# david-mathews-1994/deltarice

Measured on AMD Instinct MI355X. Metric: encode+decode GB/s (int16 in), higher is better.
Workload: dtype int16; 1 GPU; 1000000x7000 int16 Gaussian(sigma=10), m=8, 500 chunks of 2000x7000 per GPU, encode then decode, HBM resident; waveforms_per_gpu=1000000, wave_len=7000, rice_m=8, chunks_per_gpu=500, decode_impl=8

## Files before the change

### deltarice_amd/csrc/drx_blocks.hip

```cpp
#include <hip/hip_runtime.h>
#include <stdint.h>
#include <type_traits>

#include "drx_device.h"
#include "drx_internal.h"
#include "drx_iir_math.h"

namespace drx {

constexpr int kBlkSegWMin = 9;
__host__ __device__ constexpr int blk_segw_plan(uint32_t k) { return k <= 4u ? 11 : (k <= 7u ? 15 : 19); }
__host__ __device__ constexpr int blk_segw_bits10(uint64_t b10) { return b10 >= 117u ? 19 : (b10 >= 82u ? 15 : (b10 >= 54u ? 11 : 9)); }
__host__ __device__ constexpr uint32_t blk_lane_cap(int segw) { return segw <= 11 ? 76u : (segw == 15 ? 68u : 60u); }
constexpr uint32_t kBlkPre = 8;
constexpr uint32_t kBlkGuessBits = 128;
constexpr uint32_t kBlkRounds = 8;
constexpr uint32_t kBlkTail = 4;

template <int NT, int SW>
struct BlkGeom {
    static constexpr int kSegW = SW;
    static constexpr uint32_t kLaneCap = blk_lane_cap(SW);
    static constexpr uint32_t kLaneStride = kLaneCap / 2u + 1u;
    static constexpr uint32_t kWords = NT * SW;
// ... 607 lines not shown
                }
            };
            const bool lane_ok = cnt <= kBlkLaneCap && todo == cnt;
            if (!wg_any(!lane_ok)) {
                constexpr int NR = (int)(kBlkLaneCap / 2u);
                uint32_t rr[NR];
                const uint32_t wmax = (uint32_t)__builtin_amdgcn_readfirstlane((int)wave_max_u32(cnt));
#pragma unroll
                for (int i = 0; i < NR; ++i) {
                    rr[i] = 0;
                    if (2u * (uint32_t)i < wmax) rr[i] = my_stage[i];
                }
                if (RESID) s_e[tid] = sum;
                blk_barrier();
                const uint32_t base16 = RESID ? 0u : (acc_base + pre_s + incl_s - sum) & 0xffffu;
                typedef uint16_t u16x2 __attribute__((ext_vector_type(2)));
                const u16x2 b2 = {(uint16_t)base16, (uint16_t)base16};
                uint16_t *const op = obuf + (a0 + rel0);
                {
                    const uint32_t o = a0 + rel0;
                    const bool odd = (o & 1u) != 0u;
                    uint32_t *const dp = reinterpret_cast<uint32_t *>(obuf) + (o >> 1);
                    const uint32_t sel = odd ? 0x05040302u : 0x07060504u;
                    const uint32_t lim = cnt == 0u ? 0u : (odd ? cnt : cnt - 1u);
                    uint32_t prevp = RESID ? (tid ? s_e[tid - 1u] << 16 : 0u) : __builtin_bit_cast(uint32_t, b2);
#pragma unroll
                    for (int i = 0; i < NR; ++i) {
                        if (2u * (uint32_t)i < wmax) {
                            const uint32_t cur = __builtin_bit_cast(uint32_t, (u16x2)(__builtin_bit_cast(u16x2, rr[i]) + b2));
                            const uint32_t d = __builtin_amdgcn_perm(cur, prevp, sel);
                            if (2u * (uint32_t)i < lim) dp[i] = d;
                            prevp = cur;
                        }
                    }
                    if (cnt != 0u) op[cnt - 1u] = (uint16_t)(base16 + sum);
                }
                blk_barrier();
                if (FUSE) iir_lds(a0, blk_count);
                copy_out(0u);
            } else {
                uint32_t c = 0, acc = acc_base + pre_s + incl_s - sum;
                Qp = C - (todo ? f : B0);
                for (uint32_t R0 = 0; R0 < blk_count; R0 += BG::kOutCap) {
                    const uint32_t cmax = (rel0 >= R0 + BG::kOutCap) ? 0u : ((todo < R0 + BG::kOutCap - rel0) ? todo : R0 + BG::kOutCap - rel0);
                    uint16_t *outp = obuf + (int32_t)(a0 + rel0 - R0);
                    blk_parse<kBlkValue, RESID>(W, k, c < cmax, Qp, 0u, c, acc, cmax, outp);
                    blk_barrier();
                    if (FUSE) iir_lds(a0, (blk_count - R0 < BG::kOutCap) ? blk_count - R0 : BG::kOutCap);
                    copy_out(R0);
                    blk_barrier();
                }
            }
            if (FUSE && last_of_run && tid == 0u)
                __hip_atomic_store(xstate + sidx, (1ull << 63) | (uint64_t)(xs.x & 0xffffu) | ((uint64_t)(xs.y & 0xffffu) << 16) | ((uint64_t)(xs.z & 0xffffu) << 32),
                                   __ATOMIC_RELAXED, __HIP_MEMORY_SCOPE_AGENT);
            blk_barrier();
        }
        if (next_unit >= total_units) return;
        unit = next_unit;
        cur = nxt;
    }
}

static int nt_for_len(uint32_t wave_len, uint32_t k) {
    const uint64_t typ_words = ((uint64_t)wave_len * (2u * k + 7u)) >> 6;
    return typ_words <= blk_words(64, k) ? 64 : (typ_words <= blk_words(128, k) ? 128 : 256);
}
static int blocks_nt(const Geom &G) { return G.uniform ? nt_for_len(G.u_wave_len, G.k) : (int)G.rag_blk_nt; }

static double blocks_weighted(uint64_t waves, uint32_t wave_len, uint32_t k, int nt) {
    const uint64_t typ_words = ((uint64_t)wave_len * (2u * k + 7u)) >> 6;
    const uint64_t bpw = (typ_words + blk_words((uint32_t)nt, k) - 1u) / blk_words((uint32_t)nt, k);
    return (double)(waves * bpw) * (bpw <= 2u ? 1.7 : 1.0);
}
static double blocks_us_of(double weighted_blocks, int nt, uint32_t k) {
    const double resident = nt == 256 ? 768.0 : (nt == 128 ? 1536.0 : 3072.0);
    const double t_blk = (nt == 256 ? 21.0 : (nt == 128 ? 28.0 : 41.0)) * (double)blk_segw_plan(k) / 11.0;
    return (double)(uint64_t)((weighted_blocks + resident - 1.0) / resident) * t_blk;
}

bool blocks_batch(const Geom &G) {
    if (G.n_taps != 0 && !G.fast_taps) return false;
    if (!G.uniform) return G.rag_blocks != 0;
    if (!(G.total_waves <= 98304u && G.u_wave_len >= 2048u)) return false;
    const int nt = blocks_nt(G);
    const uint64_t typ_words = ((uint64_t)G.u_wave_len * (2u * G.k + 7u)) >> 6;
    const uint64_t bpw = (typ_words + blk_words((uint32_t)nt, G.k) - 1u) / blk_words((uint32_t)nt, G.k);
    const double blocks_us = blocks_us_of((double)(G.total_waves * bpw), nt, G.k) * (bpw <= 2u ? 1.7 : 1.0);
    const double lanes_us = 0.06 * (double)G.u_wave_len * (double)((G.total_waves + 98303u) / 98304u);
    return blocks_us < lanes_us;
}

std::vector<uint32_t> blocks_plan_ragged(Geom &G, const ChunkDesc *d) {
    G.rag_blocks = 0;
    G.rag_blk_classes = 0;
    uint32_t max_len = 0, min_len = 0xffffffffu;
    for (uint64_t c = 0; c < G.n_chunks; ++c) {
        max_len = d[c].wave_len > max_len ? d[c].wave_len : max_len;
        min_len = d[c].wave_len < min_len ? d[c].wave_len : min_len;
    }
    if (G.total_waves > 98304u || min_len < 2048u) return {};
    const int nt = nt_for_len(max_len, G.k);
    double wb = 0;
    for (uint64_t c = 0; c < G.n_chunks; ++c) wb += blocks_weighted(d[c].n_waves, d[c].wave_len, G.k, nt);
    const double lanes_us = 0.06 * (double)max_len * (double)((G.total_waves + 98303u) / 98304u);
    if (!(blocks_us_of(wb, nt, G.k) < lanes_us)) return {};
    const uint64_t per = (max_payload_words(max_len) + blk_words_min(64u) - 1u) / blk_words_min(64u);
    if (G.total_waves * per * 12u > (1ull << 30)) return {};
    G.rag_blocks = 1u;
    G.rag_blk_nt = (uint32_t)nt;
    G.rag_blk_slots = (uint32_t)(per ? per : 1u);
    std::vector<uint32_t> list(G.total_waves);
    uint32_t n_cls = 0, at = 0;
    for (int b = 31; b >= 11; --b) {
        uint32_t cnt = 0, cls_max = 0;
        for (uint64_t c = 0; c < G.n_chunks; ++c) {
            if ((31 - __builtin_clz(d[c].wave_len)) != b) continue;
            for (uint32_t i = 0; i < d[c].n_waves; ++i) list[at + cnt++] = (uint32_t)(d[c].wave_base + i);
            cls_max = d[c].wave_len > cls_max ? d[c].wave_len : cls_max;
        }
        if (!cnt) continue;
        G.rag_blk_class_off[n_cls] = at;
        G.rag_blk_class_len[n_cls] = cls_max;
        at += cnt;
        ++n_cls;
    }
    G.rag_blk_class_off[n_cls] = at;
    G.rag_blk_classes = n_cls;
    return list;
}

uint32_t blocks_iir_tab_words() { return 3u * kRunTabWords; }
void blocks_iir_tables(const uint32_t fast_nt[3], uint32_t t0neg, uint32_t *tab) {
    iir_run_tables(fast_nt, t0neg, 76u, tab);
    iir_run_tables(fast_nt, t0neg, 68u, tab + kRunTabWords);
    iir_run_tables(fast_nt, t0neg, 60u, tab + 2u * kRunTabWords);
}

static uint32_t blocks_slots_per_wave(const Geom &G) {
    if (!G.uniform) return G.rag_blk_slots;
    const uint64_t per = (max_payload_words(G.u_wave_len) + blk_words_min(blocks_nt(G)) - 1u) / blk_words_min(blocks_nt(G));
    return (uint32_t)(per ? per : 1u);
}

constexpr uint32_t kBlkMaxClasses = 32;
struct BlkScratch {
    uint32_t *info, *fail, *suspect, *ticket, *ends;
    uint64_t *state, *xstate;
    uint64_t bytes;
};
static BlkScratch blocks_layout(const Geom &G, void *base) {
    const uint64_t W = G.total_waves, U = W * blocks_slots_per_wave(G);
    uint64_t n32 = 4u * kBlkMaxClasses + W + W + 1u;
    n32 = (n32 + 3u) & ~3ull;
    BlkScratch L;
    uint32_t *p = reinterpret_cast<uint32_t *>(base);
    L.info = p;
    L.fail = p + 4u * kBlkMaxClasses;
    L.suspect = L.fail + W;
    L.ticket = L.suspect + W;
    L.ends = p + n32;
    const uint64_t ends32 = (U + 1u) & ~1ull;
    L.state = reinterpret_cast<uint64_t *>(L.ends + ends32);
    L.xstate = L.state + U;
    L.bytes = (n32 + ends32) * 4u + 2u * U * 8u;
    return L;
}

uint64_t blocks_scratch_bytes(const Geom &G) { return blocks_batch(G) ? blocks_layout(G, nullptr).bytes : 0; }

hipError_t launch_decode_blocks(const Geom &G, const uint32_t *d_in, uint64_t in_words, const uint64_t *d_wave_off,
                                const uint32_t *d_wave_words, void *d_blk, DevStatus *d_status, int16_t *d_out,
                                const uint32_t **fail_out, const uint32_t **suspect_out, bool resid, hipStream_t s, bool *fused_out) {
    const BlkScratch L = blocks_layout(G, d_blk);
    hipError_t e = hipMemsetAsync(d_blk, 0, L.bytes, s);
    if (e != hipSuccess) return e;
    const uint32_t spw = blocks_slots_per_wave(G);
    const uint64_t b10 = G.total_samples ? 320ull * in_words / G.total_samples : 65ull;
    const int sw = blk_segw_bits10(b10);
    auto resident_of = [](int nt) { return 256u * (nt == 64 ? 12u : (nt == 128 ? 6u : 3u)); };
    auto nt_gen = [](int nt) { return nt < 128 ? 128 : nt; };
    bool fuse = resid && G.blk_iir_tab != nullptr && !(G.dbg & DRX_DBG_IIR_SEPARATE);
    if (fuse) {
        if (G.uniform) fuse = G.total_waves >= resident_of(nt_gen(blocks_nt(G)));
        else
            for (uint32_t c = 0; c < G.rag_blk_classes; ++c)
                fuse = fuse && (G.rag_blk_class_off[c + 1] - G.rag_blk_class_off[c]) >= resident_of(nt_gen(nt_for_len(G.rag_blk_class_len[c], G.k)));
    }
// ... 53 lines not shown
```

### deltarice_amd/csrc/drx_decode_kernels.hip

```cpp
#include <hip/hip_runtime.h>
#include <stdint.h>

#include <algorithm>
#include <type_traits>

#include "drx_internal.h"
#include "drx_device.h"
#include "drx_walk.h"

namespace drx {

__global__ __launch_bounds__(64) void k_decode_simple(Geom G, const uint32_t *__restrict__ in,
                                                      const uint64_t *__restrict__ wave_off,
                                                      const uint32_t *__restrict__ wave_words, DevStatus *st,
                                                      int16_t *__restrict__ out, const uint32_t *__restrict__ only) {
    const uint64_t g = (uint64_t)blockIdx.x * 64u + threadIdx.x;
    if (g >= G.total_waves) return;
    if (only && !only[g]) return;
    const WaveRef r = locate(G, g);
    const uint32_t *s = in + wave_off[g] + 1;
    const uint32_t n = wave_words[g];
    int16_t *y = out + r.sample_off;
    const uint32_t k = G.k;
    uint64_t win = 0;
// ... 94 lines not shown
                const uint32_t s2 = sacc + d;
                if (EMIT) {
                    if (act && idx + c < len) {
                        const uint32_t i = idx + c;
                        if (((i + par4) & 1u) == 0u) {
                            held = s2 & 0xffffu;
                            held_i = i;
                            holding = true;
                        } else if (holding) {
                            *reinterpret_cast<uint32_t *>(y + i - 1u) = held | (s2 << 16);
                            holding = false;
                        } else {
                            y[i] = (int16_t)(uint16_t)s2;
                        }
                    }
                }
                sacc = act ? s2 : sacc;
                Q = act ? Q + nu : Q;
                c += act ? 1u : 0u;
            }
        }
        if (EMIT && holding) y[held_i] = (int16_t)(uint16_t)held;
        const uint32_t pos = 0u - Q;
        end = pos;
        cnt = c;
        sum = sacc;
    };

    while (done < len && blk_word < n) {
#pragma unroll
        for (int rr = 0; rr < kLongSeg; ++rr) {
            const uint32_t j = tid + NT * (uint32_t)rr;
            const uint32_t wvl = (blk_word + j < n) ? src[blk_word + j] : 0u;
            const uint32_t sgm = j / kLongSeg, i = j % kLongSeg;
            col[(kLongRows - 2u - i) * NT + sgm] = wvl;
            if (i < (uint32_t)kLongOv && sgm >= 1u) col[(kLongRows - 2u - ((uint32_t)kLongSeg + i)) * NT + sgm - 1u] = wvl;
        }
        if (tid < (uint32_t)kLongOv) {
            const uint32_t wi = blk_word + NT * kLongSeg + tid;
            col[(kLongRows - 2u - ((uint32_t)kLongSeg + tid)) * NT + NT - 1u] = (wi < n) ? src[wi] : 0u;
        }
        __syncthreads();
        const uint32_t seg_word = blk_word + tid * kLongSeg;
        const uint32_t avail_bits = seg_word < n ? ((n - seg_word) > (1u << 26) ? 0xffffffffu : (n - seg_word) * 32u) : 0u;

        uint32_t start = tid == 0 ? carry_in : kLongSegBits - kLongGuessBits, end, cnt, sum;
        parse(true, start, avail_bits, std::false_type{}, 0u, 0u, end, cnt, sum);
        for (uint32_t it = 0; it < NT; ++it) {
            s_end[tid] = end;
            __syncthreads();
            const uint32_t pe = tid ? s_end[tid - 1u] : 0u;
            const uint32_t ns = tid == 0 ? carry_in : (pe >= kLongSegBits ? pe - kLongSegBits : kLongSegBits);
            const bool changed = ns != start;
            if (!__syncthreads_or(changed ? 1 : 0)) break;
            start = ns;
            uint32_t e2, c2, s2;
            parse(changed, start, avail_bits, std::false_type{}, 0u, 0u, e2, c2, s2);
            if (changed) { end = e2; cnt = c2; sum = s2; }
        }
        const uint32_t incl_c = wave_incl_scan_dpp(cnt), incl_s = wave_incl_scan_dpp(sum);
        if (lane == 63) { s_tot[0][wv] = incl_c; s_tot[1][wv] = incl_s; }
        s_end[tid] = end;
        __syncthreads();
        uint32_t pre_c = 0, pre_s = 0, tot_c = 0, tot_s = 0;
#pragma unroll
        for (int i = 0; i < kLongWaves; ++i) {
            const uint32_t tc = s_tot[0][i], ts = s_tot[1][i];
            if (i < wv) { pre_c += tc; pre_s += ts; }
            tot_c += tc;
            tot_s += ts;
        }
        const uint32_t end_last = s_end[NT - 1u];
        uint32_t e3, c3, s3;
        parse(true, start, avail_bits, std::true_type{}, done + pre_c + incl_c - cnt, acc_base + pre_s + incl_s - sum, e3, c3, s3);
        done = (tot_c > len - done) ? len : done + tot_c;
        acc_base += tot_s;
        carry_in = end_last >= kLongSegBits ? end_last - kLongSegBits : 0u;
        blk_word += NT * kLongSeg;
        __syncthreads();
    }
    if (done < len && tid == 0) atomicOr(&st->err, kErrCorrupt);
}

template <bool FUSED, bool GEN = false>
__global__ __launch_bounds__(64, 1) void k_decode_lanes(Geom G, const uint32_t *__restrict__ in, uint64_t in_words,
                                                     const uint64_t *__restrict__ chunk_word_off,
                                                     uint64_t *__restrict__ wave_off,
                                                     uint32_t *__restrict__ wave_words,
                                                     uint64_t *__restrict__ granules, uint32_t *__restrict__ ticket,
                                                     DevStatus *st, int16_t *__restrict__ out) {
    constexpr int RW = 64;
    constexpr int LW = 16;
    constexpr int T = 64;
    constexpr int GS = 16;
    constexpr int LOG_RW = 6;
    constexpr int OSW = T / 2 + 4;
    constexpr int PPS = T / 8;
    constexpr int SPI = 64 / PPS;
    constexpr int NV = LW / 4;
    constexpr uint32_t WMASK = (1u << 27) - 1u;
    constexpr uint32_t NEED_AT = GS + 2;
    static_assert(T % GS == 0 && RW - LW >= GS + 2, "round length / ring slack");
    __shared__ uint32_t ring_all[(RW + 2) * 64];
    uint32_t *const ring = ring_all + 64;
    __shared__ __attribute__((aligned(16))) uint32_t obuf[64 * OSW];
    uint64_t *tab_off = reinterpret_cast<uint64_t *>(obuf);
    uint32_t *tab_lo = obuf + 128, *tab_hi = obuf + 192;
    static_assert(64 * OSW >= 256, "tables fit in obuf");

    const int lane = lane_id();
    const uint32_t k = G.k;
    typedef uint32_t u32x4v __attribute__((ext_vector_type(4)));
    typedef u32x4v __attribute__((address_space(1))) g_uint4;
    typedef int16_t __attribute__((address_space(1))) g_i16;
    g_i16 *const outg = (g_i16 *)out;
    uint64_t g;
    bool active;
    uint32_t len = 0, n = 0;
    uint64_t S = 1, ooff = 0;
    [[maybe_unused]] const uint32_t &len_ = len;
    const uint32_t wave_idx = blockIdx.x;
    if (FUSED) {
        uint32_t tk = 0;
        if (lane == 0) tk = atomicAdd(ticket, 1u);
        tk = (uint32_t)__builtin_amdgcn_readfirstlane((int)tk);
        constexpr bool kBlockWalkFits = sizeof(ring_all) >= kWalkBlockWords * 4u && sizeof(obuf) >= kWalkHopCap * 8u;
        const bool u_short = G.uniform && G.u_wave_len <= kWalkShortLen;
        const uint32_t n_blockwalk = G.uniform ? (u_short ? (uint32_t)G.n_chunks : 0u) : G.n_short;
        const uint64_t n_chain = G.uniform ? (u_short ? 0ull : G.n_chunks) : (uint64_t)G.n_long;
        const uint32_t n_walk = n_blockwalk + (uint32_t)((n_chain + (uint32_t)kWalkChains - 1u) / (uint32_t)kWalkChains);
        if (tk < n_walk) {
            __builtin_amdgcn_s_setprio(3);
            if (tk < n_blockwalk) {
                if constexpr (kBlockWalkFits) {
                    const uint64_t c = G.uniform ? (uint64_t)tk : (uint64_t)G.walk_short[tk];
                    walk_chunk_block(G, c, in, in_words, chunk_word_off, wave_off, wave_words, granules, st, ring_all,
                                     reinterpret_cast<uint2 *>(obuf));
                }
            } else {
                walk_chunks_scalar(G, (uint64_t)(tk - n_blockwalk) * kWalkChains, G.uniform ? nullptr : G.walk_long, n_chain,
                                   in, in_words, chunk_word_off, wave_off, wave_words, granules, st);
            }
            return;
        }
        const uint64_t t2 = tk - n_walk;
        uint64_t grp = t2 / G.n_chunks, c = t2 - grp * G.n_chunks;
        uint32_t idx = (uint32_t)grp * 64u + lane;
        uint64_t gr = 0;
        if (G.uniform) {
            const uint32_t full = G.u_n_waves >> 6, rem = G.u_n_waves & 63u;
            const uint64_t t_full = (uint64_t)full * G.n_chunks;
            if (t2 < t_full) {
                active = true;
            } else {
                if (rem == 0u) return;
                const uint32_t per = 64u / rem, sub = (uint32_t)lane / rem;
                const uint64_t c0 = (t2 - t_full) * per;
                if (c0 >= G.n_chunks) return;
                c = c0 + sub;
                idx = full * 64u + ((uint32_t)lane - sub * rem);
                active = sub < per && c < G.n_chunks;
                if (!active) { c = c0; idx = 0; }
            }
            g = c * G.u_n_waves + idx;
            if (active) {
                len = (idx + 1 == G.u_n_waves) ? (G.u_n_samples - idx * G.u_wave_len) : G.u_wave_len;
                ooff = c * (uint64_t)G.u_n_samples + (uint64_t)idx * G.u_wave_len;
            }
        } else {
            const ChunkDesc d = G.chunks[c];
            if ((uint32_t)grp * 64u >= d.n_waves) return;
            active = idx < d.n_waves;
            g = d.wave_base + idx;
            if (active) {
                len = (idx + 1 == d.n_waves) ? (d.n_samples - idx * d.wave_len) : d.wave_len;
                ooff = d.sample_off + (uint64_t)idx * d.wave_len;
            }
        }
        uint32_t spins = 0;
        for (;;) {
            if (active && !(gr & kGranValid))
                gr = __hip_atomic_load(granules + g, __ATOMIC_RELAXED, __HIP_MEMORY_SCOPE_AGENT);
            if (!__any(active && !(gr & kGranValid))) break;
            __builtin_amdgcn_s_sleep(8);
            if (++spins > (1u << 24)) {
                if (lane == 0) atomicOr(&st->err, kErrInternal);
                gr |= kGranValid;
                break;
            }
        }
        if (active) {
            n = (uint32_t)(gr >> 32) & 0x7fffffffu;
            S = chunk_word_off[c] + (uint32_t)gr + 1u;
        }
    } else if (!G.uniform && G.rag_order) {
        if (wave_idx >= G.rag_groups) return;
        const uint2 e = G.rag_order[wave_idx];
        const ChunkDesc d = G.chunks[e.x];
        const uint32_t idx = e.y * 64u + (uint32_t)lane;
        active = idx < d.n_waves;
        g = d.wave_base + idx;
        if (active) {
            len = (idx + 1 == d.n_waves) ? (d.n_samples - idx * d.wave_len) : d.wave_len;
            ooff = d.sample_off + (uint64_t)idx * d.wave_len;
            S = wave_off[g] + 1u;
            n = wave_words[g];
        }
    } else {
        g = (uint64_t)wave_idx * 64u + lane;
        active = g < G.total_waves;
        if (active) {
            const WaveRef r = locate(G, g);
            len = r.len;
            ooff = r.sample_off;
            S = wave_off[g] + 1u;
            n = wave_words[g];
        }
    }
    const uint32_t phi = active ? (uint32_t)((((uintptr_t)out >> 1) + ooff) & (uint64_t)(T - 1)) : 0u;
    const uint32_t steps = wave_max_u32(len + phi);
    const uint32_t lo_max = wave_max_u32(phi);
    const uint32_t hi_min = ~wave_max_u32(~(phi + len));
    uint64_t wo_off[PPS];
    uint32_t wo_lo[PPS], wo_hi[PPS];
    tab_off[lane] = ooff - phi;
    tab_lo[lane] = phi;
    tab_hi[lane] = phi + len;
    wave_sync();
#pragma unroll
    for (int i = 0; i < PPS; ++i) {
        const int st = i * SPI + lane / PPS, p = lane % PPS;
        wo_off[i] = tab_off[st] + 8u * (uint32_t)p;
        wo_lo[i] = tab_lo[st];
        wo_hi[i] = tab_hi[st];
    }
    wave_sync();

    const uint64_t A = (S & ~(uint64_t)(RW - 1)) - (uint64_t)RW;
    const uint32_t s0 = (uint32_t)(S - A);
    const uint32_t endw = s0 + n;
    uint32_t flw = s0 & ~(uint32_t)(LW - 1);
    const bool in_vec_ok = ((uintptr_t)in & 15u) == 0;
    uint32_t *myring = ring + lane;
    typedef uint16_t __attribute__((may_alias)) u16a;
    u16a *myout = reinterpret_cast<u16a *>(obuf + lane * OSW);
    auto store16 = [&](g_i16 *dst, const uint4 &v) __attribute__((always_inline)) {
        *(g_uint4 *)dst = (u32x4v){v.x, v.y, v.z, v.w};
    };
    auto orow16 = [&](int st, int p) __attribute__((always_inline)) -> uint4 {
        return *reinterpret_cast<const uint4 *>(obuf + st * OSW + 4 * p);
    };

    auto load_piece = [&](uint4 (&v)[NV], uint32_t ahead = 0) {
        const uint64_t a = A + flw + ahead;
        if (in_vec_ok && a + (uint32_t)LW <= in_words) {
#pragma unroll
            for (int j = 0; j < NV; ++j) v[j] = *reinterpret_cast<const uint4 *>(in + a + 4 * j);
        } else {
#pragma unroll
            for (int j = 0; j < NV; ++j) {
                v[j].x = (a + 4 * j + 0 < in_words) ? in[a + 4 * j + 0] : 0u;
                v[j].y = (a + 4 * j + 1 < in_words) ? in[a + 4 * j + 1] : 0u;
                v[j].z = (a + 4 * j + 2 < in_words) ? in[a + 4 * j + 2] : 0u;
                v[j].w = (a + 4 * j + 3 < in_words) ? in[a + 4 * j + 3] : 0u;
            }
        }
    };
    auto store_piece = [&](const uint4 (&v)[NV]) {
        const uint32_t r0 = (uint32_t)RW - (flw & (uint32_t)(RW - 1));
        uint32_t *dst = myring + r0 * 64u;
#pragma unroll
        for (int j = 0; j < NV; ++j) {
            dst[-(4 * j + 0) * 64] = v[j].x; dst[-(4 * j + 1) * 64] = v[j].y;
            dst[-(4 * j + 2) * 64] = v[j].z; dst[-(4 * j + 3) * 64] = v[j].w;
        }
        if (r0 == (uint32_t)RW) {
            myring[0] = v[0].x;
            myring[-64] = v[0].y;
        }
        flw += (uint32_t)LW;
    };

    uint32_t Q = 0u - 32u * s0;
    uint32_t Q_need;
    auto set_limits = [&]() __attribute__((always_inline)) {
        const bool more = flw < endw;
        Q_need = more ? ~(32u * (flw - NEED_AT + 1u)) : Q - 0x7fffffffu;
    };
    auto sync_refill = [&]() __attribute__((always_inline)) {
        for (;;) {
            const uint32_t avail = (flw - ((~Q) >> 5)) & WMASK;
            const bool more = flw < endw;
            if (!__any(more && avail < NEED_AT)) break;
            if (more && avail <= (uint32_t)(RW - LW)) {
                uint4 v[NV];
                load_piece(v);
                store_piece(v);
            }
            wave_sync();
        }
    };

    {
        uint4 v[NV];
        for (int i = 0; i < RW / LW; ++i) {
            if (__ballot(flw < endw && flw + (uint32_t)LW <= s0 + (uint32_t)RW) == 0) break;
            if (flw < endw && flw + (uint32_t)LW <= s0 + (uint32_t)RW) {
                load_piece(v);
                store_piece(v);
            }
        }
        wave_sync();
    }
    int32_t acc = 0;
    int32_t y2 = 0, y3 = 0;
    const uint32_t nt1 = GEN ? G.fast_nt[0] & 0xffffu : 0u, nt2 = GEN ? G.fast_nt[1] & 0xffffu : 0u,
                   nt3 = GEN ? G.fast_nt[2] & 0xffffu : 0u;
    const bool t0neg = GEN && G.fast_t0neg;
    auto advance = [&](int32_t d) __attribute__((always_inline)) {
        if constexpr (GEN) {
            uint32_t a = (uint32_t)d + __umul24(nt1, (uint32_t)acc) + __umul24(nt2, (uint32_t)y2) + __umul24(nt3, (uint32_t)y3);
            if (t0neg) a = 0u - a;
            y3 = y2;
            y2 = acc;
            acc = (int32_t)a;
        } else {
            acc += d;
        }
    };

    const uint32_t hi_step = phi + len;
    uint32_t Q_end = 0;
    auto decode_group = [&](auto first_tag, auto edge_tag, int tg, uint32_t tcur) __attribute__((always_inline)) {
        constexpr bool FIRST = decltype(first_tag)::value;
        constexpr bool EDGE = decltype(edge_tag)::value;
        if (!FIRST) {
#pragma unroll
            for (int u = 0; u < GS; u += 2) {
                const uint32_t row = __builtin_amdgcn_ubfe(Q, 5u, (uint32_t)LOG_RW);
                const uint32_t *wp = myring + row * 64u;
                const uint32_t lo = wp[0], hi = wp[64], lo2 = wp[-64];
                const uint32_t winA = __builtin_amdgcn_alignbit(hi, lo, Q);
                const uint32_t winB = __builtin_amdgcn_alignbit(lo, lo2, Q);
                const uint32_t q1 = ffbh(winA);
                const uint32_t kk1 = (winA < (1u << 24)) ? 16u : k;
                const uint32_t nu1 = ~(q1 + kk1);
                const uint32_t win2 = __builtin_amdgcn_alignbit(winA, winB, nu1);
                const uint32_t q2 = ffbh(win2);
                const uint32_t kk2 = (win2 < (1u << 24)) ? 16u : k;
                const uint32_t nu2 = ~(q2 + kk2);
                if constexpr (EDGE) {
                    Q_end = (tcur + (uint32_t)u + 1u == hi_step) ? Q + nu1 : Q_end;
                    Q_end = (tcur + (uint32_t)u + 2u == hi_step) ? Q + nu1 + nu2 : Q_end;
                }
                asm("v_add3_u32 %0, %1, %2, %3" : "=v"(Q) : "v"(Q), "v"(nu1), "v"(nu2));
                const uint32_t z1 = (q1 << kk1) + __builtin_amdgcn_ubfe(winA, nu1, kk1);
                const uint32_t z2 = (q2 << kk2) + __builtin_amdgcn_ubfe(win2, nu2, kk2);
                advance((int32_t)(z1 >> 1) ^ -(int32_t)(z1 & 1u));
                const uint32_t a1 = (uint32_t)acc;
                advance((int32_t)(z2 >> 1) ^ -(int32_t)(z2 & 1u));
                *reinterpret_cast<uint32_t *>(myout + tg + u) = __builtin_amdgcn_perm((uint32_t)acc, a1, 0x05040100u);
            }
            return;
        }
#pragma unroll
        for (int u = 0; u < GS; ++u) {
            const uint32_t row = __builtin_amdgcn_ubfe(Q, 5u, (uint32_t)LOG_RW);
            const uint32_t *wp = myring + row * 64u;
            const uint32_t lo = wp[0], hi = wp[64];
            const uint32_t win = __builtin_amdgcn_alignbit(hi, lo, Q);
            const uint32_t q = ffbh(win);
            const bool esc = win < (1u << 24);
            const uint32_t kk = esc ? 16u : k;
            const uint32_t used = q + kk + 1u;
            const uint32_t rem = __builtin_amdgcn_ubfe(win, 32u - used, kk);
            const uint32_t z = (q << kk) + rem;
            const int32_t d = (int32_t)(z >> 1) ^ -(int32_t)(z & 1u);
            const bool act = (uint32_t)(tg + u) >= phi;
            const int32_t o1 = acc, o2 = y2, o3 = y3;
            advance(d);
            acc = act ? acc : o1;
            y2 = act ? y2 : o2;
            y3 = act ? y3 : o3;
            Q = act ? Q - used : Q;
            if constexpr (EDGE) Q_end = (tcur + (uint32_t)u + 1u == hi_step) ? Q : Q_end;
            myout[tg + u] = (uint16_t)acc;
        }
    };

    auto emit_masked = [&](g_i16 *dst, uint32_t lo, uint32_t hi, uint32_t t0, const uint4 &v) __attribute__((always_inline)) {
        const int p = lane % PPS;
        const uint32_t tpos = t0 + 8u * (uint32_t)p;
        if (tpos + 8u > lo && tpos < hi) {
            if (tpos >= lo && tpos + 8u <= hi) {
                *(g_uint4 *)dst = (u32x4v){v.x, v.y, v.z, v.w};
            } else {
                const uint32_t w[4] = {v.x, v.y, v.z, v.w};
#pragma unroll
                for (int j = 0; j < 8; ++j)
                    if (tpos + (uint32_t)j >= lo && tpos + (uint32_t)j < hi)
                        dst[j] = (int16_t)(w[j >> 1] >> (16 * (j & 1)));
            }
        }
    };
    auto write_out = [&](uint32_t t0) __attribute__((always_inline)) {
        if (t0 >= lo_max && t0 + T <= hi_min) {
#pragma unroll
            for (int i = 0; i < PPS; ++i) {
                const int st = i * SPI + lane / PPS, p = lane % PPS;
                const uint4 v = orow16(st, p);
                store16(outg + wo_off[i] + t0, v);
            }
        } else {
#pragma unroll
            for (int i = 0; i < PPS; ++i) {
                const int st = i * SPI + lane / PPS, p = lane % PPS;
                const uint32_t tpos = t0 + 8u * (uint32_t)p;
                if (tpos + 8u > wo_lo[i] && tpos < wo_hi[i]) emit_masked(outg + wo_off[i] + t0, wo_lo[i], wo_hi[i], t0, orow16(st, p));
            }
        }
    };

    if (steps > 0) {
#pragma unroll 1
        for (int tg = 0; tg < T; tg += GS) {
            sync_refill();
            decode_group(std::true_type{}, std::true_type{}, tg, (uint32_t)tg);
        }
        wave_sync();
        write_out(0);
        wave_sync();
    }

    auto edge_round = [&](uint32_t t0) __attribute__((always_inline)) {
#pragma unroll 1
        for (int tg = 0; tg < T; tg += GS) {
            sync_refill();
            decode_group(std::false_type{}, std::true_type{}, tg, t0 + (uint32_t)tg);
        }
        wave_sync();
        write_out(t0);
        wave_sync();
    };
    uint32_t t0 = T;
    for (; t0 < steps && !(t0 >= lo_max && t0 + T <= hi_min); t0 += T) edge_round(t0);

    const uint32_t min_words = ((uint32_t)T * (k + 1u)) >> 5;
    uint4 pv0[NV], pv1[NV];
    bool pneed0 = false, pneed1 = false;
    set_limits();
    auto group_refill = [&]() __attribute__((always_inline)) {
        if (__any((int32_t)(Q - Q_need) <= 0)) {
            uint32_t avail = (flw - ((~Q) >> 5)) & WMASK;
            if (pneed0 && avail <= (uint32_t)(RW - LW)) {
                store_piece(pv0);
                pneed0 = false;
                avail += (uint32_t)LW;
                if (pneed1 && avail <= (uint32_t)(RW - LW)) { store_piece(pv1); pneed1 = false; }
            }
            if (!pneed0 && pneed1) {
#pragma unroll
                for (int j = 0; j < NV; ++j) pv0[j] = pv1[j];
                pneed0 = true;
                pneed1 = false;
            }
            wave_sync();
            sync_refill();
            set_limits();
        }
    };
    for (; t0 + T <= hi_min && t0 < steps; t0 += T) {
#pragma unroll 1
        for (int tg = 0; tg < T; tg += GS) {
            group_refill();
            decode_group(std::false_type{}, std::false_type{}, tg, 0u);
        }
        Q_end = (t0 + (uint32_t)T == hi_step) ? Q : Q_end;
        wave_sync();
        if (pneed0) store_piece(pv0);
        if (pneed1) store_piece(pv1);
        wave_sync();
        set_limits();
        {
            const uint32_t mc = (t0 + 2u * T <= hi_min && t0 + T < steps) ? min_words : 0u;
            const uint32_t avail = (flw - ((~Q) >> 5)) & WMASK;
            pneed0 = (flw < endw) && avail + (uint32_t)LW <= (uint32_t)RW + mc;
            pneed1 = pneed0 && (flw + (uint32_t)LW < endw) && avail + 2u * (uint32_t)LW <= (uint32_t)RW + mc;
            if (pneed0) load_piece(pv0);
            if (pneed1) load_piece(pv1, (uint32_t)LW);
        }
#pragma unroll
        for (int i = 0; i < PPS; ++i) {
            const int st = i * SPI + lane / PPS, p = lane % PPS;
            const uint4 v = orow16(st, p);
            store16(outg + wo_off[i] + t0, v);
        }
        wave_sync();
    }
    if (pneed0) store_piece(pv0);
    if (pneed1) store_piece(pv1);
    wave_sync();
    for (; t0 < steps; t0 += T) edge_round(t0);
    if (active && len && (((0u - Q_end) - 32u * s0 + 31u) >> 5) != n) atomicOr(&st->err, kErrCorrupt);
}

std::vector<uint2> decode_plan_ragged(Geom &G, const ChunkDesc *d) {
    const uint64_t n = G.n_chunks;
    uint32_t max_groups = 0, max_len = 0;
    for (uint64_t c = 0; c < n; ++c) {
        max_groups = std::max(max_groups, (d[c].n_waves + 63u) / 64u);
        max_len = std::max(max_len, d[c].wave_len);
    }
    G.max_groups = max_groups;
    G.max_wave_len64 = 64ull * max_len;
    std::vector<uint32_t> by_len(n);
    for (uint64_t c = 0; c < n; ++c) by_len[c] = (uint32_t)c;
    std::stable_sort(by_len.begin(), by_len.end(), [&](uint32_t a, uint32_t b) { return d[a].wave_len > d[b].wave_len; });
    std::vector<uint2> order;
    uint64_t n_long_groups = 0;
    for (uint32_t c : by_len)
        for (uint32_t j = 0; j < (d[c].n_waves + 63u) / 64u; ++j) {
            order.push_back(make_uint2(c, j));
            if (d[c].wave_len > kWalkShortLen) ++n_long_groups;
        }
    if (order.size() <= 0x7fffffffull) {
        G.rag_groups = (uint32_t)order.size();
        G.rag_groups_long = (uint32_t)n_long_groups;
    } else {
        order.clear();
    }
    return order;
}

enum class Dec { Simple, Blocks, Long, LanesFused, Lanes, LanesSplit };
enum class Walk { None, InLaunch, Parallel, Serial };
struct DecodeRoute {
    Dec dec;
    Walk walk;
    WalkRoute par;
    bool gen;
};

static DecodeRoute route_decode(const Geom &G, int impl, bool tables_ready, bool have_pw, bool have_blk, bool have_side) {
    DecodeRoute R{};
    R.gen = G.n_taps != 0;
    R.par = route_walk(G, tables_ready, have_pw);
    const bool simple = impl == 0 || (R.gen && !G.fast_taps);
    const bool want_fused = !tables_ready && impl == 8;
    const bool blocks = !simple && !(G.dbg & (DRX_DBG_NO_LONG_PATHS | DRX_DBG_LONG_NOT_BLOCKS)) && have_blk && blocks_batch(G) && (!R.gen || (G.iir_tab && G.iir_state));
    const bool longp = !simple && !blocks && !R.gen && !(G.dbg & DRX_DBG_NO_LONG_PATHS) && G.uniform && long_waveform_batch(G.total_waves, G.u_wave_len);
    const bool sparse = !G.uniform && (uint64_t)G.n_chunks * G.max_groups > 8ull * ((G.total_waves + 63u) / 64u) + 4096ull;
    R.dec = simple ? Dec::Simple : (blocks ? Dec::Blocks : (longp ? Dec::Long : Dec::Lanes));
    const bool parallel = R.par.chunk_wide || R.par.blocks;
    if (R.dec == Dec::Lanes && want_fused && !sparse && !parallel) R.dec = Dec::LanesFused;
    R.walk = tables_ready ? Walk::None : (R.dec == Dec::LanesFused ? Walk::InLaunch : (parallel ? Walk::Parallel : Walk::Serial));
    if (R.dec == Dec::Lanes && R.par.chunk_wide && R.par.blocks && have_side && G.rag_order && G.rag_groups_long &&
        G.rag_groups_long < G.rag_groups && !(G.dbg & DRX_DBG_RAGGED_ONE_LANES_LAUNCH)) R.dec = Dec::LanesSplit;
    return R;
}

hipError_t launch_decode(const Geom &G, const uint32_t *d_in, uint64_t in_words,
                         const uint64_t *d_chunk_word_off, int16_t *d_out, uint64_t *d_wave_off,
                         uint32_t *d_wave_words, uint64_t *d_granules, DevStatus *d_status, int impl, bool tables_ready,
                         void *d_pw, void *d_blk, const SideStream *side, hipEvent_t *ev, hipStream_t s, uint32_t *path_out) {
    uint32_t path_dummy = 0;
    uint32_t &path = path_out ? *path_out : path_dummy;
    path = 0;
    if (G.total_waves == 0) return hipSuccess;
    mark(ev, 0, s);
    const DecodeRoute R = route_decode(G, impl, tables_ready, d_pw != nullptr, d_blk != nullptr, side && side->s);
    const bool gen = R.gen;
    const unsigned nb_plain = blocks_for(G.total_waves, 64);

    auto launch_lanes = [&](const Geom &Gv, unsigned nb, hipStream_t st_) {
        path |= DRX_PATH_LANES;
        if (gen)
            k_decode_lanes<false, true><<<nb, 64, 0, st_>>>(Gv, d_in, in_words, d_chunk_word_off, d_wave_off, d_wave_words, nullptr, nullptr, d_status, d_out);
        else
            k_decode_lanes<false><<<nb, 64, 0, st_>>>(Gv, d_in, in_words, d_chunk_word_off, d_wave_off, d_wave_words, nullptr, nullptr, d_status, d_out);
    };

    if (R.walk == Walk::InLaunch) {
        hipError_t e = hipMemsetAsync(d_granules, 0, (G.total_waves + 2) * sizeof(uint64_t), s);
        if (e != hipSuccess) return e;
    } else if (R.walk == Walk::Parallel) {
        const bool split = R.dec == Dec::LanesSplit;
        hipError_t e = walk_scratch_reset(G, d_pw, s);
        if (e != hipSuccess) return e;
        const bool forked = R.par.chunk_wide && R.par.blocks && side && side->s;
        hipStream_t spw = forked ? side->s : s;
        if (forked) {
            if ((e = hipEventRecord(side->fork, s)) != hipSuccess) return e;
            if ((e = hipStreamWaitEvent(side->s, side->fork, 0)) != hipSuccess) return e;
        }
        if (R.par.chunk_wide)
            launch_walk_chunk_wide(G, d_in, in_words, d_chunk_word_off, d_wave_off, d_wave_words, d_status, d_pw, R.par.by_chains, spw);
        if (split) {
            Geom Gl = G;
            Gl.rag_groups = G.rag_groups_long;
            launch_lanes(Gl, Gl.rag_groups, spw);
        }
        if (forked && (e = hipEventRecord(side->join, side->s)) != hipSuccess) {
            (void)hipStreamSynchronize(side->s);
            return e;
        }
        if (R.par.blocks) launch_walk_blocks(G, d_in, in_words, d_chunk_word_off, d_wave_off, d_wave_words, d_status, d_pw, s);
        if (split) {
            mark(ev, 1, s);
            Geom Gs = G;
            Gs.rag_order = G.rag_order + G.rag_groups_long;
            Gs.rag_groups = G.rag_groups - G.rag_groups_long;
            launch_lanes(Gs, Gs.rag_groups, s);
        }
        if (forked && (e = hipStreamWaitEvent(s, side->join, 0)) != hipSuccess) {
            (void)hipStreamSynchronize(side->s);
            return e;
        }
    } else if (R.walk == Walk::Serial) {
        launch_walk_serial(G, d_in, in_words, d_chunk_word_off, d_wave_off, d_wave_words, d_status, s);
    }
    if (R.dec != Dec::LanesSplit) mark(ev, 1, s);

    switch (R.dec) {
    case Dec::LanesFused: {
        uint32_t *ticket = reinterpret_cast<uint32_t *>(d_granules + G.total_waves);
        unsigned n_walk, groups;
        unsigned nb;
        if (G.uniform) {
            n_walk = (G.u_wave_len <= kWalkShortLen) ? (unsigned)G.n_chunks : blocks_for(G.n_chunks, kWalkChains);
            groups = (G.u_n_waves + 63u) / 64u;
            const uint32_t full = G.u_n_waves >> 6, rem = G.u_n_waves & 63u;
            nb = n_walk + (unsigned)(G.n_chunks * full) + (rem ? (unsigned)((G.n_chunks + 64u / rem - 1u) / (64u / rem)) : 0u);
        } else {
            n_walk = G.n_short + blocks_for(G.n_long, kWalkChains);
            groups = G.max_groups;
            nb = n_walk + (unsigned)(G.n_chunks * groups);
        }
        path |= DRX_PATH_LANES_FUSED;
        if (gen)
            k_decode_lanes<true, true><<<nb, 64, 0, s>>>(G, d_in, in_words, d_chunk_word_off, d_wave_off, d_wave_words, d_granules, ticket, d_status, d_out);
        else
            k_decode_lanes<true><<<nb, 64, 0, s>>>(G, d_in, in_words, d_chunk_word_off, d_wave_off, d_wave_words, d_granules, ticket, d_status, d_out);
        break;
    }
    case Dec::Blocks: {
        const uint32_t *fail = nullptr, *suspect = nullptr;
        bool fused = false;
        hipError_t e = launch_decode_blocks(G, d_in, in_words, d_wave_off, d_wave_words, d_blk, d_status, d_out, &fail, &suspect, gen, s, &fused);
        if (e != hipSuccess) return e;
        path |= DRX_PATH_BLOCKS | (gen ? (fused ? DRX_PATH_IIR_FUSED : DRX_PATH_IIR) : 0u);
        k_decode_long<<<(unsigned)G.total_waves, kLongThreads, 0, s>>>(G, d_in, d_wave_off, d_wave_words, d_status, d_out, fail, suspect, gen ? 1u : 0u);
        if (gen) {
            if (!fused && (e = launch_iir(G, G.iir_chunk_tile_base, G.iir_n_tiles, G.iir_tab, G.iir_state, fail, d_status, d_out, s)) != hipSuccess) return e;
            k_decode_simple<<<nb_plain, 64, 0, s>>>(G, d_in, d_wave_off, d_wave_words, d_status, d_out, fail);
        }
        break;
    }
    case Dec::Long:
        path |= DRX_PATH_LONG;
        k_decode_long<<<(unsigned)G.total_waves, kLongThreads, 0, s>>>(G, d_in, d_wave_off, d_wave_words, d_status, d_out, nullptr, nullptr, 0u);
        break;
    case Dec::Lanes:
// ... 16 lines not shown
```

### deltarice_amd/csrc/drx_internal.h

```cpp
#ifndef DRX_INTERNAL_H
#define DRX_INTERNAL_H

#include <hip/hip_runtime.h>
#include <stdint.h>

#include <vector>

#include "../../include/deltarice_hip.h"

namespace drx {

struct ChunkDesc {
    uint64_t sample_off;
    uint64_t wave_base;
    uint32_t n_samples;
    uint32_t wave_len;
    uint32_t n_waves;
    uint32_t pad_;
};

struct Geom {
    const ChunkDesc *chunks;
    uint64_t n_chunks;
    uint64_t total_waves;
    uint32_t uniform;
    uint32_t u_n_samples, u_wave_len, u_n_waves;
    uint32_t k;
    uint32_t n_taps;
    const int32_t *taps;
    uint32_t fast_taps, fast_t0neg;
    uint32_t fast_nt[3];
    uint32_t enc_fast;
    uint32_t enc_t[4];
    uint64_t total_samples;
    uint64_t *host_words;
    uint32_t dbg;
    const uint32_t *walk_short, *walk_long;
    uint32_t n_short, n_long, max_groups;
    uint64_t max_wave_len64;
    uint32_t rag_blocks, rag_blk_nt, rag_blk_slots;
    const uint32_t *rag_blk_list;
    uint32_t rag_blk_classes;
    uint32_t rag_blk_class_off[33], rag_blk_class_len[32];
    const uint32_t *iir_tab;
    const uint32_t *blk_iir_tab;
    const uint64_t *iir_chunk_tile_base;
    uint64_t iir_n_tiles;
    uint64_t *iir_state;
    const uint64_t *seg_unit_base;
    uint64_t seg_units;
    uint32_t rag_par, rag_bw_blocks_max;
    uint32_t rag_bw_min_len;
    uint32_t rag_pw_min_waves;
    const uint2 *rag_order;
    uint32_t rag_groups;
    uint32_t rag_groups_long;
    const uint32_t *pc_wg_base;
    uint32_t pc_super;
    uint32_t pc_packed;
};

struct DevStatus {
    uint32_t err;
    uint32_t pad_;
    uint64_t total_words;
};

constexpr uint32_t kErrCapacity = 1u;
constexpr uint32_t kErrCorrupt = 2u;
constexpr uint32_t kErrInternal = 4u;

hipError_t launch_encode(const Geom &G, const int16_t *d_in, uint32_t *d_out, uint64_t out_cap,
                         uint64_t *d_chunk_word_off, uint32_t *d_wave_words, uint32_t *d_wave_rel,
                         uint64_t *d_chunk_words, DevStatus *d_status, hipEvent_t *ev, hipStream_t s);

__host__ __device__ inline bool long_waveform_batch(uint64_t total_waves, uint32_t wave_len) {
    return (wave_len >= 65536u && total_waves <= 16384u) || (wave_len >= 16384u && total_waves <= 4096u);
}
static inline unsigned blocks_for(uint64_t items, unsigned per_block) { return (unsigned)((items + per_block - 1) / per_block); }
static inline void mark(hipEvent_t *ev, int i, hipStream_t s) {
    if (ev) (void)hipEventRecord(ev[i], s);
}

inline uint64_t chunk_max_words(uint32_t n_samples, uint32_t n_waves) { return 1u + 2ull * n_waves + (((uint64_t)n_samples * 25u + 31u) >> 5); }

struct WalkRoute {
    bool chunk_wide, blocks;
    bool by_chains;
};
WalkRoute route_walk(const Geom &G, bool tables_ready, bool have_scratch);
std::vector<uint32_t> walk_plan_ragged(Geom &G, const ChunkDesc *host_chunks);
uint64_t walk_scratch_bytes(const Geom &G);
hipError_t walk_scratch_reset(const Geom &G, void *d_pw, hipStream_t s);
void launch_walk_chunk_wide(const Geom &G, const uint32_t *d_in, uint64_t in_words, const uint64_t *d_chunk_word_off,
                            uint64_t *d_wave_off, uint32_t *d_wave_words, DevStatus *d_status, void *d_pw, bool by_chains, hipStream_t s);
void launch_walk_blocks(const Geom &G, const uint32_t *d_in, uint64_t in_words, const uint64_t *d_chunk_word_off,
                        uint64_t *d_wave_off, uint32_t *d_wave_words, DevStatus *d_status, void *d_pw, hipStream_t s);
void launch_walk_serial(const Geom &G, const uint32_t *d_in, uint64_t in_words, const uint64_t *d_chunk_word_off,
                        uint64_t *d_wave_off, uint32_t *d_wave_words, DevStatus *d_status, hipStream_t s);
hipError_t launch_sideband_tables(const Geom &G, const uint32_t *d_in, uint64_t in_words, const uint64_t *d_chunk_word_off,
                                  const uint32_t *d_n, uint64_t *d_wave_off, uint32_t *d_wave_words, DevStatus *d_status, hipStream_t s,
                                  const uint32_t *d_list = nullptr, uint32_t n_list = 0);
int select_walk_class(uint32_t n_waves, uint32_t wave_len);
hipError_t launch_select_walk(const Geom &G, const uint32_t *d_in, uint64_t in_words, const uint64_t *d_chunk_word_off,
                              const uint32_t *d_lists, uint32_t n_sparse, uint32_t n_block, uint32_t n_chain, uint32_t *d_fail,
                              uint64_t *d_wave_off, uint32_t *d_wave_words, DevStatus *d_status, hipStream_t s);
hipError_t launch_decode_select(const Geom &G, const uint32_t *d_in, const uint64_t *d_wave_off, const uint32_t *d_wave_words,
                                const uint64_t *d_sel, uint64_t n_sel, DevStatus *d_status, int16_t *d_out, uint64_t stride,
                                hipStream_t s);
uint64_t gather_scan_blocks(uint64_t n_sel);
hipError_t launch_gather(const Geom &G, const uint32_t *d_in, const uint64_t *d_wave_off, const uint32_t *d_wave_words,
                         const uint64_t *d_sel, uint64_t n_sel, uint64_t chunk_waves, const uint32_t *d_chunk_samples,
                         uint32_t *d_out, uint64_t out_cap, uint64_t *d_out_chunk_off, uint32_t *d_out_wave_words,
                         uint32_t *d_ent_words, uint64_t *d_ent_pos, uint64_t *d_block_sum, uint32_t *d_ctrl, bool tiles,
                         uint64_t mean_words, bool resume, DevStatus *d_status, hipEvent_t *ev, hipStream_t s);
hipError_t launch_estimate_words(const Geom &G, const int16_t *d_in, unsigned long long *d_words16, hipStream_t s);

hipError_t launch_encode_fused(const Geom &G, int wide, const int16_t *d_in, uint32_t *d_out, uint64_t out_cap,
                               uint64_t *d_chunk_word_off, uint32_t *d_wave_words, uint64_t *d_scan,
                               DevStatus *d_status, hipEvent_t *ev, hipStream_t s);

constexpr uint32_t kEsRingWords = 2496;
constexpr uint64_t kEsMinUnits = 8192;
hipError_t launch_encode_stream(const Geom &G, const int16_t *d_in, uint32_t *d_out, uint64_t out_cap,
                                uint64_t *d_chunk_word_off, uint32_t *d_wave_words, uint64_t *d_scan,
                                DevStatus *d_status, hipEvent_t *ev, hipStream_t s);

constexpr uint32_t kEsSegWaves = 4;
constexpr uint32_t kEsSegMinLen = 1024, kEsSegMaxLen = 7168;
struct EsSegShape { uint32_t seg_len, nseg, tpw; };
__host__ __device__ inline EsSegShape es_seg_shape(uint32_t L, uint32_t seg_target) {
    EsSegShape sh;
    uint32_t n = (L + seg_target - 1u) / seg_target;
    n = n ? n : 1u;
    const uint32_t dn = n / kEsSegWaves * kEsSegWaves, up = (n + kEsSegWaves - 1u) / kEsSegWaves * kEsSegWaves;
    n = up;
    if (dn && dn != up) {
        const uint64_t sd = (L + dn - 1u) / dn, su = (L + up - 1u) / up;
        const uint64_t pen_dn = sd > seg_target ? (sd - seg_target) * 55u : 0u, pen_up = su < seg_target ? (seg_target - su) * 40u : 0u;
        if (sd * 57u <= (uint64_t)seg_target * 67u && pen_dn < pen_up) n = dn;
    }
    sh.seg_len = (((L + n - 1u) / n) + 7u) & ~7u;
    sh.nseg = (L + sh.seg_len - 1u) / sh.seg_len;
    sh.tpw = (sh.nseg + kEsSegWaves - 1u) / kEsSegWaves;
    return sh;
}
inline bool stream_segs_admits(const Geom &G) { return G.uniform && (G.n_taps == 0 || G.enc_fast) && G.u_wave_len >= 64u &&
                                                       G.total_waves * es_seg_shape(G.u_wave_len, kEsSegMinLen).tpw < 0xffff0000ull; }
constexpr uint32_t kEsSegsFromLen = 20480;
inline uint64_t segs_scan_words(const Geom &G, uint32_t seg_target) { return 3 * G.total_waves * es_seg_shape(G.u_wave_len, seg_target).tpw + 192; }
hipError_t launch_encode_stream_segs(const Geom &G, uint32_t seg_target, const int16_t *d_in, uint32_t *d_out, uint64_t out_cap,
                                     uint64_t *d_chunk_word_off, uint32_t *d_wave_words, uint64_t *d_scan,
                                     DevStatus *d_status, hipEvent_t *ev, hipStream_t s);

bool long_batch_admits(const Geom &G);
bool long_batch(const Geom &G);
uint64_t long_batch_units(const Geom &G);
std::vector<uint64_t> segments_plan_ragged(Geom &G, const ChunkDesc *host_chunks);
// ... 110 lines not shown
```

Measured before the change: 1488 GB/s.

## Stage decoded lanes output in registers to shrink LDS and raise occupancy

Adds a STAGED variant of the lanes decode kernel. In the interior rounds it keeps decoded sample pairs in a register array and flushes them through a 16-row LDS transposition buffer in four passes, which shrinks the shared-memory footprint. Edge rounds write each 16-sample group out directly. The launch bound now requests more waves per CU, and the blocks-vs-lanes routing threshold is recomputed from the new in-flight lane count (256 CUs × 8 waves × 64). Higher occupancy should hide memory latency better. The costs are extra wave syncs, more register pressure from the staging array, and smaller per-group global stores on edges.

```diff
diff --git a/deltarice_amd/csrc/drx_blocks.hip b/deltarice_amd/csrc/drx_blocks.hip
--- a/deltarice_amd/csrc/drx_blocks.hip
+++ b/deltarice_amd/csrc/drx_blocks.hip
@@ -713,12 +713,12 @@
 bool blocks_batch(const Geom &G) {
     if (G.n_taps != 0 && !G.fast_taps) return false;
     if (!G.uniform) return G.rag_blocks != 0;
-    if (!(G.total_waves <= 98304u && G.u_wave_len >= 2048u)) return false;
+    if (!(G.total_waves <= kLanesInFlight && G.u_wave_len >= 2048u)) return false;
     const int nt = blocks_nt(G);
     const uint64_t typ_words = ((uint64_t)G.u_wave_len * (2u * G.k + 7u)) >> 6;
     const uint64_t bpw = (typ_words + blk_words((uint32_t)nt, G.k) - 1u) / blk_words((uint32_t)nt, G.k);
     const double blocks_us = blocks_us_of((double)(G.total_waves * bpw), nt, G.k) * (bpw <= 2u ? 1.7 : 1.0);
-    const double lanes_us = 0.06 * (double)G.u_wave_len * (double)((G.total_waves + 98303u) / 98304u);
+    const double lanes_us = 0.06 * (double)G.u_wave_len * (double)((G.total_waves + kLanesInFlight - 1u) / kLanesInFlight);
     return blocks_us < lanes_us;
 }
 
@@ -730,11 +730,11 @@
         max_len = d[c].wave_len > max_len ? d[c].wave_len : max_len;
         min_len = d[c].wave_len < min_len ? d[c].wave_len : min_len;
     }
-    if (G.total_waves > 98304u || min_len < 2048u) return {};
+    if (G.total_waves > kLanesInFlight || min_len < 2048u) return {};
     const int nt = nt_for_len(max_len, G.k);
     double wb = 0;
     for (uint64_t c = 0; c < G.n_chunks; ++c) wb += blocks_weighted(d[c].n_waves, d[c].wave_len, G.k, nt);
-    const double lanes_us = 0.06 * (double)max_len * (double)((G.total_waves + 98303u) / 98304u);
+    const double lanes_us = 0.06 * (double)max_len * (double)((G.total_waves + kLanesInFlight - 1u) / kLanesInFlight);
     if (!(blocks_us_of(wb, nt, G.k) < lanes_us)) return {};
     const uint64_t per = (max_payload_words(max_len) + blk_words_min(64u) - 1u) / blk_words_min(64u);
     if (G.total_waves * per * 12u > (1ull << 30)) return {};
diff --git a/deltarice_amd/csrc/drx_decode_kernels.hip b/deltarice_amd/csrc/drx_decode_kernels.hip
--- a/deltarice_amd/csrc/drx_decode_kernels.hip
+++ b/deltarice_amd/csrc/drx_decode_kernels.hip
@@ -200,8 +200,8 @@
     if (done < len && tid == 0) atomicOr(&st->err, kErrCorrupt);
 }
 
-template <bool FUSED, bool GEN = false>
-__global__ __launch_bounds__(64, 1) void k_decode_lanes(Geom G, const uint32_t *__restrict__ in, uint64_t in_words,
+template <bool FUSED, bool GEN = false, bool STAGED = false>
+__global__ __launch_bounds__(64, STAGED ? kLanesWavesPerCU / 4 : 1) void k_decode_lanes(Geom G, const uint32_t *__restrict__ in, uint64_t in_words,
                                                      const uint64_t *__restrict__ chunk_word_off,
                                                      uint64_t *__restrict__ wave_off,
                                                      uint32_t *__restrict__ wave_words,
@@ -221,10 +221,14 @@
     static_assert(T % GS == 0 && RW - LW >= GS + 2, "round length / ring slack");
     __shared__ uint32_t ring_all[(RW + 2) * 64];
     uint32_t *const ring = ring_all + 64;
-    __shared__ __attribute__((aligned(16))) uint32_t obuf[64 * OSW];
-    uint64_t *tab_off = reinterpret_cast<uint64_t *>(obuf);
-    uint32_t *tab_lo = obuf + 128, *tab_hi = obuf + 192;
-    static_assert(64 * OSW >= 256, "tables fit in obuf");
+    static_assert(!(FUSED && STAGED), "the in-launch block walker borrows the whole transposition buffer");
+    constexpr int OROWS = STAGED ? 16 : 64;
+    constexpr int EGW = GS / 2;
+    constexpr int TAB0 = STAGED ? OROWS * OSW : 0;
+    __shared__ __attribute__((aligned(16))) uint32_t obuf[STAGED ? OROWS * OSW + 256 : 64 * OSW];
+    uint64_t *tab_off = reinterpret_cast<uint64_t *>(obuf + TAB0);
+    uint32_t *tab_lo = obuf + TAB0 + 128, *tab_hi = obuf + TAB0 + 192;
+    static_assert(64 * OSW >= 256 && OROWS * OSW >= 64 * EGW && (TAB0 & 3) == 0, "tables / an edge group fit in obuf");
 
     const int lane = lane_id();
     const uint32_t k = G.k;
@@ -341,18 +345,20 @@
     const uint32_t hi_min = ~wave_max_u32(~(phi + len));
     uint64_t wo_off[PPS];
     uint32_t wo_lo[PPS], wo_hi[PPS];
-    tab_off[lane] = ooff - phi;
+    tab_off[lane] = STAGED ? (uint64_t)(uintptr_t)out + 2u * (ooff - phi) : ooff - phi;
     tab_lo[lane] = phi;
     tab_hi[lane] = phi + len;
     wave_sync();
-#pragma unroll
-    for (int i = 0; i < PPS; ++i) {
-        const int st = i * SPI + lane / PPS, p = lane % PPS;
-        wo_off[i] = tab_off[st] + 8u * (uint32_t)p;
-        wo_lo[i] = tab_lo[st];
-        wo_hi[i] = tab_hi[st];
-    }
-    wave_sync();
+    if constexpr (!STAGED) {
+#pragma unroll
+        for (int i = 0; i < PPS; ++i) {
+            const int st = i * SPI + lane / PPS, p = lane % PPS;
+            wo_off[i] = tab_off[st] + 8u * (uint32_t)p;
+            wo_lo[i] = tab_lo[st];
+            wo_hi[i] = tab_hi[st];
+        }
+        wave_sync();
+    }
 
     const uint64_t A = (S & ~(uint64_t)(RW - 1)) - (uint64_t)RW;
     const uint32_t s0 = (uint32_t)(S - A);
@@ -361,7 +367,7 @@
     const bool in_vec_ok = ((uintptr_t)in & 15u) == 0;
     uint32_t *myring = ring + lane;
     typedef uint16_t __attribute__((may_alias)) u16a;
-    u16a *myout = reinterpret_cast<u16a *>(obuf + lane * OSW);
+    u16a *myout = reinterpret_cast<u16a *>(obuf + lane * (STAGED ? EGW : OSW));
     auto store16 = [&](g_i16 *dst, const uint4 &v) __attribute__((always_inline)) {
         *(g_uint4 *)dst = (u32x4v){v.x, v.y, v.z, v.w};
     };
@@ -449,7 +455,10 @@
 
     const uint32_t hi_step = phi + len;
     uint32_t Q_end = 0;
-    auto decode_group = [&](auto first_tag, auto edge_tag, int tg, uint32_t tcur) __attribute__((always_inline)) {
+    auto to_lds = [&](int tg, int u, uint32_t pk) __attribute__((always_inline)) {
+        *reinterpret_cast<uint32_t *>(myout + (STAGED ? 0 : tg) + u) = pk;
+    };
+    auto decode_group = [&](auto first_tag, auto edge_tag, int tg, uint32_t tcur, auto &&put_pair) __attribute__((always_inline)) {
         constexpr bool FIRST = decltype(first_tag)::value;
         constexpr bool EDGE = decltype(edge_tag)::value;
         if (!FIRST) {
@@ -477,7 +486,7 @@
                 advance((int32_t)(z1 >> 1) ^ -(int32_t)(z1 & 1u));
                 const uint32_t a1 = (uint32_t)acc;
                 advance((int32_t)(z2 >> 1) ^ -(int32_t)(z2 & 1u));
-                *reinterpret_cast<uint32_t *>(myout + tg + u) = __builtin_amdgcn_perm((uint32_t)acc, a1, 0x05040100u);
+                put_pair(tg, u, __builtin_amdgcn_perm((uint32_t)acc, a1, 0x05040100u));
             }
             return;
         }
@@ -502,13 +511,11 @@
             y3 = act ? y3 : o3;
             Q = act ? Q - used : Q;
             if constexpr (EDGE) Q_end = (tcur + (uint32_t)u + 1u == hi_step) ? Q : Q_end;
-            myout[tg + u] = (uint16_t)acc;
-        }
-    };
-
-    auto emit_masked = [&](g_i16 *dst, uint32_t lo, uint32_t hi, uint32_t t0, const uint4 &v) __attribute__((always_inline)) {
-        const int p = lane % PPS;
-        const uint32_t tpos = t0 + 8u * (uint32_t)p;
+            myout[(STAGED ? 0 : tg) + u] = (uint16_t)acc;
+        }
+    };
+
+    auto emit_masked = [&](g_i16 *dst, uint32_t lo, uint32_t hi, uint32_t tpos, const uint4 &v) __attribute__((always_inline)) {
         if (tpos + 8u > lo && tpos < hi) {
             if (tpos >= lo && tpos + 8u <= hi) {
                 *(g_uint4 *)dst = (u32x4v){v.x, v.y, v.z, v.w};
@@ -534,8 +541,39 @@
             for (int i = 0; i < PPS; ++i) {
                 const int st = i * SPI + lane / PPS, p = lane % PPS;
                 const uint32_t tpos = t0 + 8u * (uint32_t)p;
-                if (tpos + 8u > wo_lo[i] && tpos < wo_hi[i]) emit_masked(outg + wo_off[i] + t0, wo_lo[i], wo_hi[i], t0, orow16(st, p));
-            }
+                if (tpos + 8u > wo_lo[i] && tpos < wo_hi[i]) emit_masked(outg + wo_off[i] + t0, wo_lo[i], wo_hi[i], tpos, orow16(st, p));
+            }
+        }
+    };
+    auto write_group = [&](uint32_t tq) __attribute__((always_inline)) {
+#pragma unroll
+        for (int i = 0; i < 2; ++i) {
+            const int st = i * 32 + lane / 2, p = lane % 2;
+            const uint32_t tpos = tq + 8u * (uint32_t)p;
+            const uint32_t lo = tab_lo[st], hi = tab_hi[st];
+            if (tpos + 8u > lo && tpos < hi)
+                emit_masked((g_i16 *)(uintptr_t)tab_off[st] + tpos, lo, hi, tpos, *reinterpret_cast<const uint4 *>(obuf + st * EGW + 4 * p));
+        }
+    };
+    auto flush_staged = [&](uint32_t t0, const uint32_t (&stage)[T / 2]) __attribute__((always_inline)) {
+        static_assert(SPI * 2 == OROWS || !STAGED, "two store instructions per slice");
+        uint32_t *const put = obuf + (lane & (OROWS - 1)) * OSW;
+        const uint32_t *const get = obuf + (lane / PPS) * OSW + 4 * (lane % PPS);
+        const uint32_t adv = 2u * (t0 + 8u * (uint32_t)(lane % PPS));
+#pragma unroll
+        for (int s = 0; s < 64 / OROWS; ++s) {
+            if (lane / OROWS == s) {
+#pragma unroll
+                for (int j = 0; j < T / 2; ++j) put[j] = stage[j];
+            }
+            wave_sync();
+#pragma unroll
+            for (int h = 0; h < 2; ++h) {
+                const int i = 2 * s + h;
+                const u32x4v v = *reinterpret_cast<const u32x4v *>(get + h * SPI * OSW);
+                *(g_uint4 *)(uintptr_t)(tab_off[i * SPI + lane / PPS] + adv) = v;
+            }
+            wave_sync();
         }
     };
 
@@ -543,22 +581,36 @@
 #pragma unroll 1
         for (int tg = 0; tg < T; tg += GS) {
             sync_refill();
-            decode_group(std::true_type{}, std::true_type{}, tg, (uint32_t)tg);
-        }
-        wave_sync();
-        write_out(0);
-        wave_sync();
+            decode_group(std::true_type{}, std::true_type{}, tg, (uint32_t)tg, to_lds);
+            if constexpr (STAGED) {
+                wave_sync();
+                write_group((uint32_t)tg);
+                wave_sync();
+            }
+        }
+        if constexpr (!STAGED) {
+            wave_sync();
+            write_out(0);
+            wave_sync();
+        }
     }
 
     auto edge_round = [&](uint32_t t0) __attribute__((always_inline)) {
 #pragma unroll 1
         for (int tg = 0; tg < T; tg += GS) {
             sync_refill();
-            decode_group(std::false_type{}, std::true_type{}, tg, t0 + (uint32_t)tg);
-        }
-        wave_sync();
-        write_out(t0);
-        wave_sync();
+            decode_group(std::false_type{}, std::true_type{}, tg, t0 + (uint32_t)tg, to_lds);
+            if constexpr (STAGED) {
+                wave_sync();
+                write_group(t0 + (uint32_t)tg);
+                wave_sync();
+            }
+        }
+        if constexpr (!STAGED) {
+            wave_sync();
+            write_out(t0);
+            wave_sync();
+        }
     };
     uint32_t t0 = T;
     for (; t0 < steps && !(t0 >= lo_max && t0 + T <= hi_min); t0 += T) edge_round(t0);
@@ -588,10 +640,23 @@
         }
     };
     for (; t0 + T <= hi_min && t0 < steps; t0 += T) {
+        uint32_t stage[T / 2];
+        if constexpr (STAGED) {
+            auto to_stage = [&](int tg, int u, uint32_t pk) __attribute__((always_inline)) {
+                asm volatile("" : "+v"(pk));
+                stage[(tg + u) >> 1] = pk;
+            };
+#pragma unroll
+            for (int tg = 0; tg < T; tg += GS) {
+                group_refill();
+                decode_group(std::false_type{}, std::false_type{}, tg, 0u, to_stage);
+            }
+        } else {
 #pragma unroll 1
-        for (int tg = 0; tg < T; tg += GS) {
-            group_refill();
-            decode_group(std::false_type{}, std::false_type{}, tg, 0u);
+            for (int tg = 0; tg < T; tg += GS) {
+                group_refill();
+                decode_group(std::false_type{}, std::false_type{}, tg, 0u, to_lds);
+            }
         }
         Q_end = (t0 + (uint32_t)T == hi_step) ? Q : Q_end;
         wave_sync();
@@ -607,13 +672,17 @@
             if (pneed0) load_piece(pv0);
             if (pneed1) load_piece(pv1, (uint32_t)LW);
         }
-#pragma unroll
-        for (int i = 0; i < PPS; ++i) {
-            const int st = i * SPI + lane / PPS, p = lane % PPS;
-            const uint4 v = orow16(st, p);
-            store16(outg + wo_off[i] + t0, v);
-        }
-        wave_sync();
+        if constexpr (STAGED) {
+            flush_staged(t0, stage);
+        } else {
+#pragma unroll
+            for (int i = 0; i < PPS; ++i) {
+                const int st = i * SPI + lane / PPS, p = lane % PPS;
+                const uint4 v = orow16(st, p);
+                store16(outg + wo_off[i] + t0, v);
+            }
+            wave_sync();
+        }
     }
     if (pneed0) store_piece(pv0);
     if (pneed1) store_piece(pv1);
@@ -693,9 +762,9 @@
     auto launch_lanes = [&](const Geom &Gv, unsigned nb, hipStream_t st_) {
         path |= DRX_PATH_LANES;
         if (gen)
-            k_decode_lanes<false, true><<<nb, 64, 0, st_>>>(Gv, d_in, in_words, d_chunk_word_off, d_wave_off, d_wave_words, nullptr, nullptr, d_status, d_out);
+            k_decode_lanes<false, true, true><<<nb, 64, 0, st_>>>(Gv, d_in, in_words, d_chunk_word_off, d_wave_off, d_wave_words, nullptr, nullptr, d_status, d_out);
         else
-            k_decode_lanes<false><<<nb, 64, 0, st_>>>(Gv, d_in, in_words, d_chunk_word_off, d_wave_off, d_wave_words, nullptr, nullptr, d_status, d_out);
+            k_decode_lanes<false, false, true><<<nb, 64, 0, st_>>>(Gv, d_in, in_words, d_chunk_word_off, d_wave_off, d_wave_words, nullptr, nullptr, d_status, d_out);
     };
 
     if (R.walk == Walk::InLaunch) {
diff --git a/deltarice_amd/csrc/drx_internal.h b/deltarice_amd/csrc/drx_internal.h
--- a/deltarice_amd/csrc/drx_internal.h
+++ b/deltarice_amd/csrc/drx_internal.h
@@ -74,6 +74,9 @@
                          uint64_t *d_chunk_word_off, uint32_t *d_wave_words, uint32_t *d_wave_rel,
                          uint64_t *d_chunk_words, DevStatus *d_status, hipEvent_t *ev, hipStream_t s);
 
+constexpr int kLanesWavesPerCU = 8;
+constexpr uint64_t kLanesInFlight = 256ull * kLanesWavesPerCU * 64ull;
+
 __host__ __device__ inline bool long_waveform_batch(uint64_t total_waves, uint32_t wave_len) {
     return (wave_len >= 65536u && total_waves <= 16384u) || (wave_len >= 16384u && total_waves <= 4096u);
 }
```

Result: slower. 1470 GB/s (-1.2%).
